# genomewalker/metadamage

Measured on AMD Instinct MI355X. Metric: TaxID damage fits/sec, higher is better.
Workload: dtype f64

## Files before the change

metadamage_amd/csrc/mdfit.hip:

```cpp
#include <hip/hip_runtime.h>

#include <algorithm>
#include <cmath>
#include <cstdint>
#include <cstdlib>
#include <cstdio>
#include <cstring>
#include <mutex>

#include "../../include/mdfit.h"
#include "mdfit_hpdi.h"
#include "mdfit_host.h"
#include "mdfit_laplace.h"
#include "mdfit_mappsis.h"
#include "mdfit_model.h"
#include "mdfit_primitive.h"
#include "mdfit_special.h"

#ifdef MDFIT_DEV_HPTIME
__device__ unsigned long long* g_dev_hpt = nullptr;
#define MDFIT_DEV_T(idx) \
  do {                     \
    if (g_dev_hpt != nullptr) g_dev_hpt[(idx)] = __builtin_amdgcn_s_memrealtime(); \
  } while (0)
#endif

namespace mdfit {

constexpr int kAll = 0, kFR = 1;

__device__ __forceinline__ double* diag(double* out, int64_t taxon, int sub) {
  return out + taxon * MDFIT_NOUT + MDFIT_F_DIAG + MDFIT_DIAG_STRIDE * sub;
}

__device__ __forceinline__ double sel4(const double v[4], int j) {
  return j == 0 ? v[0] : (j == 1 ? v[1] : (j == 2 ? v[2] : v[3]));
}

#ifdef MDFIT_STAMP
__device__ unsigned long long* g_stamp = nullptr;
__device__ __forceinline__ unsigned long long stamp() {
  __builtin_amdgcn_sched_barrier(0);
  unsigned long long t = __builtin_amdgcn_s_memtime();
  __builtin_amdgcn_sched_barrier(0);
  return t;
}
#endif

constexpr int kWsReady = 8, kWsClaim = 9, kWsStarted = 10, kWsBad = 11;
constexpr int kWsEarlyClaimed = 12;
constexpr int kWsDefRes = 32, kWsDefDone = 33, kWsDefClaim = 34, kWsEarlyQuit = 35;
constexpr unsigned kDefClosed = 0x40000000u;
constexpr int kReadyStride = 6;
static_assert(kReadyStride == MDFIT_NSUBFIT, "K0 zeroes the ready list with one thread per (taxon, sub-fit)");
__device__ __forceinline__ void ready_put(uint64_t* f, double v) {
  __hip_atomic_store(f, ~(uint64_t)__double_as_longlong(isnan(v) ? NAN : v), __ATOMIC_RELAXED,
                     __HIP_MEMORY_SCOPE_AGENT);
}
__device__ __forceinline__ uint64_t ready_get(const uint64_t* f) {
  return __hip_atomic_load(f, __ATOMIC_RELAXED, __HIP_MEMORY_SCOPE_AGENT);
}
constexpr int kHpdiCtr = 16;

__device__ __forceinline__ int kpos(int i) { return i < kNHalf ? i : i - kNHalf; }

__global__ __launch_bounds__(256) void init_kernel(const uint32_t* __restrict__ gy,
                                                   const uint32_t* __restrict__ gN, int64_t T,
                                                   double* __restrict__ out, int* __restrict__ ws) {
  const int64_t i = (int64_t)blockIdx.x * blockDim.x + threadIdx.x;
  if (i < 64) ws[i] = 0;
  if (i < MDFIT_NSUBFIT * T) reinterpret_cast<double*>(reinterpret_cast<char*>(ws) + 256)[i] = 0.0;
  if (i >= MDFIT_NSUBFIT * T) return;
  const int64_t taxon = i / MDFIT_NSUBFIT;
  const int sub = (int)(i % MDFIT_NSUBFIT);
  const bool pmd = sub == 0 || sub == 2 || sub == 3;
  const int lo = (sub == 3 || sub == 5) ? kNHalf : 0;
  const int hi = sub < 2 ? kNPos : lo + kNHalf;
  double s[8] = {0, 0, 0, 0, 0, 0, 0, 0};
  for (int c = lo; c < hi; ++c) {
    const double y = (double)gy[taxon * kLD + c], N = (double)gN[taxon * kLD + c];
    const int k = kpos(c);
    s[0] += y;
    s[1] += N;
    if (k == 0) { s[2] += y; s[3] += N; }
    if (k == 1) { s[4] += y; s[5] += N; }
    if (k >= 9) { s[6] += y; s[7] += N; }
  }
  double u0[4];
  u0[3] = flog(100.0);
  if (!pmd) {
    u0[0] = logit(clampd((s[0] + 0.5) / (s[1] + 1.0), 1e-4, 0.9));
    u0[1] = u0[2] = 0.0;
  } else {
    const double c0 = clampd((s[6] + 0.5) / (s[7] + 1.0), 1e-4, 0.3);
    const double r1 = (s[2] + 0.5) / (s[3] + 1.0);
    const double r2 = (s[4] + 0.5) / (s[5] + 1.0);
    const double A0 = clampd(r1 - c0, 1e-3, 0.9 * (1.0 - c0));
    double q0 = 1.0 / 3.0;
    if (r1 - c0 > 1e-3) q0 = clampd(1.0 - (r2 - c0) / (r1 - c0), 0.05, 0.95);
    u0[0] = logit(q0);
    u0[1] = logit(A0);
    u0[2] = c0;
  }
  double* dg = diag(out, taxon, sub);
#pragma unroll
  for (int j = 0; j < 4; ++j) dg[j] = u0[j];
}

#ifndef MDFIT_FIT_WAVES_PER_EU
#define MDFIT_FIT_WAVES_PER_EU 2
#endif


constexpr int kIdle = 0, kAllFit = 1, kPairFit = 2, kNextPair = 3;
constexpr int kPrioEvals = 15;

constexpr unsigned kEscIndef = 1u, kEscProbe = 2u, kEscNc = 4u, kEscExhOk = 8u, kEscN = 16u, kEscCount = 0x70u,
                   kEscRescued = 0x100u, kEscRelax = 0x200u, kEscPolish = 0x400u, kEscPolishProbe = 0x800u,
                   kEscGrad = 0x1000u, kEscGradProbe = 0x2000u, kEscGradN = 0x4000u, kEscGradCount = 0x3C000u;


struct HpdiIO {
  const uint32_t* gN;
// ... 38 lines not shown
  __shared__ int s_b[2];
  bool wide = false;
  hpdi::WideRec rec;
  if (valid) {
    double lo = NAN, hi = NAN;
    if (!skip) wide = !hpdi::prep_position(N, a, b, lo, hi, rec);
    if (!wide) hpdi_write<kFit>(io, item, N, lo, hi);
  }
  bool near = false;
  if (wide) {
    const double tau = sqrt(rec.sd * rec.sd + (rec.mu - rec.m) * (rec.mu - rec.m));
    near = rec.m < 1.5 * tau || rec.N - rec.m < 1.5 * tau;
  }
  const int w = (int)threadIdx.x / kWave, ln = (int)threadIdx.x % kWave;
  const unsigned long long mf = __ballot(wide && near), mb = __ballot(wide && !near);
  if (ln == 0) {
    s_n[0][w] = __popcll(mf);
    s_n[1][w] = __popcll(mb);
  }
  __syncthreads();
  if (threadIdx.x == 0) {
    int tf = 0, tb = 0;
#pragma unroll
    for (int k = 0; k < kW; ++k) {
      tf += s_n[0][k];
      tb += s_n[1][k];
    }
    s_b[0] = tf ? atomicAdd(ctr, tf) : 0;
    s_b[1] = tb ? atomicAdd(ctr + 2, tb) : 0;
  }
  __syncthreads();
  if (wide) {
    int bf = s_b[0], bb = s_b[1];
    for (int k = 0; k < w; ++k) {
      bf += s_n[0][k];
      bb += s_n[1][k];
    }
    rec.item = item;
    const unsigned long long below = (1ull << ln) - 1ull;
    const int64_t slot = near ? (int64_t)(bf + __popcll(mf & below)) : n_items - 1 - (bb + __popcll(mb & below));
    recs[slot] = rec;
  }
}

__device__ __forceinline__ double tree8(const double* x) {
  return ((x[0] + x[1]) + (x[2] + x[3])) + ((x[4] + x[5]) + (x[6] + x[7]));
}
__device__ __forceinline__ double tree16(const double* x) { return tree8(x) + tree8(x + 8); }

template <int PPL>
__global__ __launch_bounds__(kWave) __attribute__((amdgpu_waves_per_eu(MDFIT_FIT_WAVES_PER_EU)))
void fit_kernel(const uint32_t* __restrict__ gy, const uint32_t* __restrict__ gN, int64_t T,
                int max_iter, double tol, double* __restrict__ out, int* __restrict__ ws,
                double* __restrict__ ready, int base_prio) {
  static_assert(PPL == 1 || PPL == 2, "points per lane");
  constexpr int kSlot = PPL == 1 ? 32 : 16;
  constexpr int kHalf = kSlot / 2;
  const int lane = threadIdx.x;
  const int r = lane & (kSlot - 1);
  const int h = r / kHalf;
  const int jh = r & (kHalf - 1);
  const int leader = lane & ~(kSlot - 1);
  const unsigned long long slot_mask = (kSlot == 32 ? 0xFFFFFFFFull : 0xFFFFull) << leader;
  const int qi = blockIdx.x % kQueues;
  const int64_t tl = T * qi / kQueues, nq = T * (qi + 1) / kQueues - tl;

  PointData pa, pb;
  int vA_all, vA_pair, vB_all = 0, vB_pair = 0;
  int kA_all, kA_pair, kB_all = 0, kB_pair = 0, colA_all;
  if (PPL == 1) {
    const int i = r & 15;
    vA_all = vA_pair = i < kNHalf;
    kA_all = kA_pair = vA_all ? i : 0;
    colA_all = vA_all ? h * kNHalf + i : 0;
  } else {
    vA_all = vB_all = r < kNHalf;
    kA_all = kB_all = vA_all ? r : 0;
    colA_all = vA_all ? r : 0;
    kA_pair = 2 * jh;
    kB_pair = 2 * jh + 1;
    vA_pair = true;
    vB_pair = kB_pair < kNHalf;
    kB_pair = vB_pair ? kB_pair : 0;
  }
  const int srcA = leader + (PPL == 2 ? kA_pair : 0);
  const int srcB = leader + (PPL == 2 ? (vB_pair ? kB_pair : 0) : 0);
  pa.y = pa.N = pb.y = pb.N = 0.0;
  pa.valid = vA_all;
  pa.k = kA_all;
  pb.valid = vB_all;
  pb.k = kB_all;
  pa.pmd = pb.pmd = true;

  __shared__ __attribute__((aligned(16))) double sAcc[kNAcc][kWave + 2];
  __shared__ __attribute__((aligned(16))) double sSum[2][kWave];
  if (blockIdx.x == 0 && lane == 0)
    __hip_atomic_store(ws + kWsStarted, 1, __ATOMIC_RELAXED, __HIP_MEMORY_SCOPE_AGENT);
  int mode = kIdle;
  int drained = 0, allok = 0;
  int64_t taxon = 0;
  int sub = 0;
  int running = 0;
  double u[4] = {0, 0, 0, 0}, ut[4] = {0, 0, 0, 0}, d[4] = {0, 0, 0, 0};
  double curF = INFINITY, curMag = 0.0, curPg = 0.0, t = 1.0;
  double curG3 = 0.0, curGd = 0.0;
  unsigned esc = 0u;
  int evals = 0, status = MDFIT_MAXITER;
  int first = 1;
#ifdef MDFIT_STAMP
  unsigned long long st_eval = 0, st_red = 0, st_logic = 0, st_fetch = 0, st_trips = 0;
  unsigned long long st_claim1 = 0, st_claim2 = 0;
  const unsigned long long k0 = stamp();
#endif

  while (true) {
#ifdef MDFIT_STAMP
    const unsigned long long f0 = stamp();
#endif
    bool starting = false;
    const bool need1 = mode == kIdle && !drained;
#ifdef MDFIT_STAMP
    const unsigned long long a0 = stamp();
#endif
    if (__any(need1)) {
      const unsigned long long m = __ballot(need1 && r == 0);
      int base = 0;
      if (lane == 0) base = atomicAdd(ws + qi, __popcll(m));
      base = __shfl(base, 0);
      if (need1) {
        const int64_t task = (int64_t)base + __popcll(m & ((1ull << leader) - 1ull));
        if (task >= 2 * nq) {
          drained = true;
        } else {
          sub = task < nq ? 0 : 1;
          taxon = tl + task - (sub ? nq : 0);
          mode = kAllFit;
          starting = true;
          pa.pmd = pb.pmd = sub == 0;
          pa.valid = vA_all;
          pa.k = kA_all;
          pa.y = pa.valid ? (double)gy[taxon * kLD + colA_all] : 0.0;
          pa.N = pa.valid ? (double)gN[taxon * kLD + colA_all] : 0.0;
          if (PPL == 2) {
            pb.valid = vB_all;
            pb.k = kB_all;
            pb.y = pb.valid ? (double)gy[taxon * kLD + kNHalf + colA_all] : 0.0;
            pb.N = pb.valid ? (double)gN[taxon * kLD + kNHalf + colA_all] : 0.0;
          }
          const double* dg = diag(out, taxon, sub);
#pragma unroll
          for (int j = 0; j < 4; ++j) u[j] = dg[j];
        }
      }
    }
#ifdef MDFIT_STAMP
    const unsigned long long a1 = stamp();
#ifndef MDFIT_STAMP2
    st_claim1 += a1 - a0;
#endif
#endif
    const bool next = mode == kNextPair;
    if (__any(next)) {
      if (PPL == 2) {
        const double ya = __shfl(pa.y, srcA), Na = __shfl(pa.N, srcA);
        const double yb = __shfl(pb.y, srcA), Nb = __shfl(pb.N, srcA);
        const double ya2 = __shfl(pa.y, srcB), Na2 = __shfl(pa.N, srcB);
        const double yb2 = __shfl(pb.y, srcB), Nb2 = __shfl(pb.N, srcB);
        if (next) {
          pa.valid = vA_pair;
          pa.k = kA_pair;
          pa.y = h ? yb : ya;
          pa.N = h ? Nb : Na;
          pb.valid = vB_pair;
          pb.k = kB_pair;
          pb.y = vB_pair ? (h ? yb2 : ya2) : 0.0;
          pb.N = vB_pair ? (h ? Nb2 : Na2) : 0.0;
        }
      }
      if (next) {
        sub = (pa.pmd ? 2 : 4) + h;
        mode = kPairFit;
        starting = true;
        if (!allok) {
          const double* dg = diag(out, taxon, sub);
#pragma unroll
          for (int j = 0; j < 4; ++j) u[j] = dg[j];
        }
      }
    }
#if defined(MDFIT_STAMP) && !defined(MDFIT_STAMP2)
    st_claim2 += stamp() - a1;
#endif
    if (starting) {
#pragma unroll
      for (int j = 0; j < 4; ++j) ut[j] = u[j];
      curF = INFINITY;
      curMag = curPg = 0.0;
      esc = 0u;
      t = 1.0;
      evals = 0;
      status = MDFIT_MAXITER;
      first = true;
      running = true;
    }
    if (!__any(mode != kIdle || !drained)) break;
#ifdef MDFIT_STAMP
    const unsigned long long e0 = stamp();
#endif
    if (!__any(running)) continue;

    const bool whole = mode == kAllFit;
    const Theta th = make_theta<kHalf>(pa.pmd, ut);
    double acc[kNAcc];
#pragma unroll
    for (int j = 0; j < kNAcc; ++j) acc[j] = 0.0;
    const int accf = (esc & kEscPolish) != 0u;
    const bool null_wave = !__any(running && pa.pmd != 0);
    const bool whole_wave = !__any(running && !whole);
    if (PPL == 1) {
      point_accum<true>(pa, th, acc, accf, null_wave, whole_wave);
    } else {
      const bool src15 = whole || h == 1;
      auto pad3 = [&](const LG3& v) -> LG3 { return src15 ? rowb3<15>(v) : rowb3<7>(v); };
      const PointArgs gb = point_args(pb, th);
      const LG3 t3b = lg3<true>(pb.N + th.phi);
      const LG3 t6 = pad3(t3b);
      const LG3 tb1 = lg3<true>(pb.y + gb.a);
      const LG3 tb2 = lg3<true>(pb.N - pb.y + gb.b);
      LG3 tb4, tb5;
      if (null_wave) {
        tb4 = pad3(tb1);
        tb5 = pad3(tb2);
      } else {
        tb4 = lg3<true>(gb.a);
        tb5 = lg3<true>(gb.b);
      }
      double accb[kNAcc];
#pragma unroll
      for (int j = 0; j < kNAcc; ++j) accb[j] = 0.0;
      point_finish(pb, th, gb, tb1, tb2, t3b, tb4, tb5, t6, accb, accf);
      const PointArgs ga = point_args(pa, th);
      const LG3 ta3 = lg3<true>(pa.N + th.phi);
      const LG3 ta1 = lg3<true>(pa.y + ga.a);
      const LG3 ta2 = lg3<true>(pa.N - pa.y + ga.b);
      LG3 ta4 = tb4, ta5 = tb5;
      if (!null_wave && !whole_wave) {
        ta4 = lg3<true>(ga.a);
        ta5 = lg3<true>(ga.b);
      }
      point_finish(pa, th, ga, ta1, ta2, ta3, ta4, ta5, t6, acc, accf);
#pragma unroll
      for (int j = 0; j < kNAcc; ++j) acc[j] = opaque(acc[j]) + opaque(accb[j]);
    }
#ifdef MDFIT_STAMP
    const unsigned long long e1 = stamp();
#endif
#pragma unroll
    for (int j = 0; j < kNAcc; ++j) sAcc[j][lane] = acc[j];
    __syncthreads();
    if (PPL == 1) {
      const double* a = &sAcc[jh][leader + 16 * h];
      const double* b = &sAcc[jh][leader + 16 * (1 - h)];
      double x[16];
#pragma unroll
      for (int k = 0; k < 16; ++k) {
        const double ak = a[k], bk = b[k];
        x[k] = whole ? ak + bk : ak;
      }
      sSum[0][lane] = tree16(x);
      __syncthreads();
      const double* src = &sSum[0][leader + 16 * h];
#pragma unroll
      for (int j = 0; j < kNAcc; ++j) acc[j] = src[j];
// ... 165 lines not shown
                                                     : (i == 6 ? (double)status : ((esc & kEscPolish) ? 1.0 : 0.0))));
          diag(out, taxon, sub)[i] = v;
        }
        allok = status == MDFIT_OK;
        running = false;
      }
    }
    if (__any(running && evals >= 2 * kPrioEvals)) __builtin_amdgcn_s_setprio(3);
    else if (__any(running && evals >= kPrioEvals)) __builtin_amdgcn_s_setprio(2);
    else if (base_prio) __builtin_amdgcn_s_setprio(1);
    else __builtin_amdgcn_s_setprio(0);
    const unsigned long long busy = __ballot(running);
    if ((busy & slot_mask) == 0ull) {
      if (mode == kAllFit) {
        if (sub == 0) {
          auto sig = [](double v) {
            const double e = exp(-fabs(v));
            const double rr = rcp(1.0 + e);
            return v >= 0.0 ? rr : e * rr;
          };
          const bool badA = vA_all && pa.y > pa.N;
          const bool badB = PPL == 2 && vB_all && pb.y > pb.N;
          const bool bad = (__ballot(badA || badB) & slot_mask) != 0ull;
          if (r == 0) {
#ifdef MDFIT_DEV_HPTIME
            MDFIT_DEV_T(taxon);
#endif
            const int idx = atomicAdd(ws + kWsReady, 1);
            uint64_t* e = reinterpret_cast<uint64_t*>(ready + (int64_t)idx * kReadyStride);
            ready_put(e + 0, bad ? NAN : sig(u[0]));
            ready_put(e + 1, bad ? NAN : sig(u[1]));
            ready_put(e + 2, bad ? NAN : u[2]);
            ready_put(e + 3, bad ? NAN : exp(u[3]) + 2.0);
            __hip_atomic_store(e + 4, ~(uint64_t)taxon, __ATOMIC_RELAXED, __HIP_MEMORY_SCOPE_AGENT);
          }
        }
        mode = kNextPair;
      } else if (mode == kPairFit) {
#ifdef MDFIT_DEV_HPTIME
        if (r == 0) MDFIT_DEV_T(T + taxon);
#endif
        mode = kIdle;
      }
    }
#ifdef MDFIT_STAMP
    const unsigned long long l1 = stamp();
    st_fetch += e0 - f0;
    st_eval += e1 - e0;
    st_red += e2 - e1;
    st_logic += l1 - e2;
    st_trips += 1;
#endif
  }
#ifdef MDFIT_STAMP
  if (lane == 0 && g_stamp != nullptr) {
    unsigned long long* rr = g_stamp + (int64_t)blockIdx.x * 8;
    rr[0] = st_eval;
    rr[1] = st_red;
    rr[2] = st_logic;
    rr[3] = st_fetch;
    rr[4] = st_trips;
    rr[5] = stamp() - k0;
    rr[6] = st_claim1;
    rr[7] = st_claim2;
  }
#endif
}


__device__ __forceinline__ double predict_median(double A, double q, double c, int k, double N) {
  if (N == 0.0) return NAN;
  return fmin(fma(A, powk(1.0 - q, k), c), 1.0);
}

template <int G>
__device__ __forceinline__ double nsigma_group(bool valid, double lP, double lN, double n) {
  const double v = valid ? 1.0 : 0.0;
  const double dd0 = v * ((-2.0 * lP) - (-2.0 * lN));
  const double md = gsum<G>(dd0) / n;
  const double wP = gsum<G>(v * (-2.0 * lP));
  const double wN = gsum<G>(v * (-2.0 * lN));
  const double dd = v * (dd0 - md);
  const double var = gsum<G>(dd * dd) / n;
  return (wN - wP) / sqrt(n * var);
}

__device__ __forceinline__ Theta sel(bool c, const Theta& a, const Theta& b) {
  Theta r;
  r.q = c ? a.q : b.q;
  r.omq = c ? a.omq : b.omq;
  r.iomq = c ? a.iomq : b.iomq;
  r.A = c ? a.A : b.A;
  r.JA = c ? a.JA : b.JA;
  r.c = c ? a.c : b.c;
  r.iomc = c ? a.iomc : b.iomc;
  r.delta = c ? a.delta : b.delta;
  r.phi = c ? a.phi : b.phi;
  r.lprior = c ? a.lprior : b.lprior;
  return r;
}

__device__ __forceinline__ double read_lane(double v, int l) {
  return __hiloint2double(__builtin_amdgcn_readlane(__double2hiint(v), l),
                          __builtin_amdgcn_readlane(__double2loint(v), l));
}
__device__ __forceinline__ Theta read_theta(const Theta& t, int l) {
// ... 512 lines not shown
    }
  }
}

__global__ __launch_bounds__(kWave) void objective_kernel(
    const int32_t* __restrict__ model, const int32_t* __restrict__ subset,
    const uint32_t* __restrict__ gy, const uint32_t* __restrict__ gN, const double* __restrict__ gu,
    int64_t n, double* __restrict__ F, double* __restrict__ g, double* __restrict__ H,
    double* __restrict__ ell_out) {
  const int64_t i = blockIdx.x;
  if (i >= n) return;
  if (threadIdx.x < kNPos) ell_out[i * kNPos + threadIdx.x] = 0.0;
  __syncthreads();
  double u[4];
#pragma unroll
  for (int j = 0; j < 4; ++j) u[j] = gu[i * 4 + j];
  const bool pmd = model[i] == 0;
  if (subset[i] == 0) objective_group<kAll>(gy, gN, i, pmd, false, u, F, g, H, ell_out);
  else objective_group<kFR>(gy, gN, i, pmd, subset[i] == 2, u, F, g, H, ell_out);
}

}

namespace mdfit::host {
thread_local char g_err[512] = "";

int set_err(int code, const char* msg) {
  std::snprintf(g_err, sizeof(g_err), "%s", msg);
  return code;
}

int check_launch(const char* what) {
  hipError_t e = hipGetLastError();
  if (e != hipSuccess) {
    std::snprintf(g_err, sizeof(g_err), "%s: %s", what, hipGetErrorString(e));
    return (int)e;
  }
  g_err[0] = '\0';
  return 0;
}
}

namespace {
using mdfit::host::check_launch;
using mdfit::host::fit_grid;
using mdfit::host::g_err;
using mdfit::host::set_err;

constexpr int kProfMax = 256;
constexpr int64_t kPpl2MinTaxa = 13000;
constexpr int64_t kStreamMaxTaxa = 60000;
constexpr int64_t kDeferCap = 131072;
int64_t defer_cap(int64_t n_taxa) { return std::min<int64_t>(n_taxa * mdfit::kNPos, kDeferCap); }
struct ProfState {
  bool on = false;
  bool fit_only = false;
  int n = 0;
  hipEvent_t ev[kProfMax][4];
  bool made = false;
};
ProfState g_prof;

void prof_record(int slot, hipStream_t s) {
  if (g_prof.fit_only && (slot == 0 || slot == 3)) return;
  if (g_prof.on && g_prof.n < kProfMax) (void)hipEventRecord(g_prof.ev[g_prof.n][slot], s);
}
}

namespace {
int env_int(const char* name, int dflt) {
  const char* e = std::getenv(name);
  return e ? std::atoi(e) : dflt;
}

double* ready_buf(void* ws) { return reinterpret_cast<double*>(static_cast<char*>(ws) + 256); }
mdfit::hpdi::WideRec* hpdi_recs(void* ws) {
  return reinterpret_cast<mdfit::hpdi::WideRec*>(static_cast<char*>(ws) + 256);
}
mdfit::hpdi::WideRec* hpdi_recs_after_ready(void* ws, int64_t n_taxa) {
  return reinterpret_cast<mdfit::hpdi::WideRec*>(static_cast<char*>(ws) + 256 +
                                                 n_taxa * mdfit::kReadyStride * (int64_t)sizeof(double));
}

struct Fork {
  hipStream_t s[2] = {nullptr, nullptr};
  hipEvent_t fork[2] = {nullptr, nullptr}, join[2] = {nullptr, nullptr};
  bool ok = false;
  std::mutex mu;
};
Fork* side_fork() {
  constexpr int kMaxDev = 64;
  static Fork f[kMaxDev];
  static std::mutex make_mu;
  int dev = 0;
  if (hipGetDevice(&dev) != hipSuccess || dev < 0 || dev >= kMaxDev) return nullptr;
  Fork& x = f[dev];
  std::lock_guard<std::mutex> g(make_mu);
  if (!x.ok) {
    bool ok = true;
    for (int k = 0; k < 2 && ok; ++k)
      ok = (x.s[k] != nullptr || hipStreamCreateWithFlags(&x.s[k], hipStreamNonBlocking) == hipSuccess) &&
           (x.fork[k] != nullptr || hipEventCreateWithFlags(&x.fork[k], hipEventDisableTiming) == hipSuccess) &&
           (x.join[k] != nullptr || hipEventCreateWithFlags(&x.join[k], hipEventDisableTiming) == hipSuccess);
    if (!ok) return nullptr;
    x.ok = true;
  }
// ... 50 lines not shown
#endif

int mdfit_profile_enable(int on) {
  if (on && !g_prof.made) {
    for (int i = 0; i < kProfMax; ++i)
      for (int j = 0; j < 4; ++j)
        if (hipEventCreate(&g_prof.ev[i][j]) != hipSuccess) return set_err(MDFIT_E_HIP, "hipEventCreate");
    g_prof.made = true;
  }
  g_prof.on = on != 0;
  g_prof.fit_only = on == 2;
  g_prof.n = 0;
  return 0;
}

int mdfit_profile_read(double* call_ms, double* fit_ms, int32_t* n_calls) {
  if (!call_ms || !fit_ms || !n_calls) return set_err(MDFIT_E_ARG, "null argument");
  double a = 0.0, b = 0.0;
  for (int i = 0; i < g_prof.n; ++i) {
    float x = 0.f, y = 0.f;
    if (hipEventSynchronize(g_prof.ev[i][2]) != hipSuccess ||
        (!g_prof.fit_only && (hipEventSynchronize(g_prof.ev[i][3]) != hipSuccess ||
                              hipEventElapsedTime(&x, g_prof.ev[i][0], g_prof.ev[i][3]) != hipSuccess)) ||
        hipEventElapsedTime(&y, g_prof.ev[i][1], g_prof.ev[i][2]) != hipSuccess)
      return set_err(MDFIT_E_HIP, "hipEventElapsedTime");
    a += x;
    b += y;
  }
  *call_ms = g_prof.fit_only ? -1.0 : a;
  *fit_ms = b;
  *n_calls = g_prof.n;
  g_prof.n = 0;
  return 0;
}

void mdfit_default_opts(mdfit_opts* o) {
  if (!o) return;
  std::memset(o, 0, sizeof(*o));
  o->mode = MDFIT_MODE_MAP;
  o->max_iter = 200;
  o->tol_step = 1e-9;
  o->seed = 0;
  o->num_warmup = 500;
  o->num_samples = 1000;
  o->index_base = 0;
}

int64_t mdfit_workspace_bytes(int64_t n_taxa, const mdfit_opts* opts) {
  if (n_taxa < 0) return 0;
  mdfit_opts o;
  mdfit_default_opts(&o);
  if (opts) o = *opts;
  if (o.mode == MDFIT_MODE_NUTS) return mdfit::nuts::workspace_bytes(n_taxa, o.num_samples);
  return 256 + n_taxa * mdfit::kReadyStride * (int64_t)sizeof(double) +
         (n_taxa >= kStreamMaxTaxa ? n_taxa * mdfit::kNPos * (int64_t)sizeof(mdfit::hpdi::WideRec) : 0) +
         defer_cap(n_taxa) * (int64_t)sizeof(int);
}

int mdfit_fit_batch(const uint32_t* y, const uint32_t* N, const uint32_t* mm, int64_t n_taxa,
                    const mdfit_opts* opts, double* out, float* pred, int32_t* status,
                    void* workspace, void* hip_stream) {
  if (n_taxa < 0) return set_err(MDFIT_E_ARG, "n_taxa < 0");
  if (n_taxa == 0) return 0;
  if (!y || !N || !out || !status) return set_err(MDFIT_E_ARG, "null required pointer");
  if (!workspace) return set_err(MDFIT_E_ARG, "workspace (mdfit_workspace_bytes() bytes) required");
  mdfit_opts o;
  mdfit_default_opts(&o);
  if (opts) o = *opts;
  if (o.mode != MDFIT_MODE_MAP && o.mode != MDFIT_MODE_NUTS) return set_err(MDFIT_E_ARG, "unsupported mode");
  if (o.max_iter < 1) return set_err(MDFIT_E_ARG, "max_iter < 1");
  if (n_taxa > ((int64_t)1 << 25)) return set_err(MDFIT_E_ARG, "n_taxa exceeds 2^25 per call");
  hipStream_t s = (hipStream_t)hip_stream;
  int* ws = (int*)workspace;
  prof_record(0, s);
  if (o.mode == MDFIT_MODE_NUTS) {
    if (hipMemsetAsync(ws, 0, 256, s) != hipSuccess) return check_launch("hipMemsetAsync(workspace)");
    if (int rc = mdfit::nuts::fit_batch(y, N, mm, n_taxa, o, out, pred, status, workspace, s)) return rc;
    prof_record(3, s);
    if (g_prof.on && g_prof.n < kProfMax) ++g_prof.n;
    return 0;
  }
  const int64_t n_init = MDFIT_NSUBFIT * n_taxa;
  mdfit::host::debug_poison(s);
  hipLaunchKernelGGL(mdfit::init_kernel, dim3((unsigned)((n_init + 255) / 256)), dim3(256), 0, s, y, N,
                     n_taxa, out, ws);
  if (int rc = check_launch("init_kernel")) return rc;
  int ppl = n_taxa >= kPpl2MinTaxa ? 2 : 1;
  if (const char* e = std::getenv("MDFIT_FIT_PPL")) ppl = std::atoi(e) == 2 ? 2 : 1;
  const int per = pred != nullptr ? mdfit::kNPos : 1;
  const int64_t n_items = n_taxa * per;
  double* ready = ready_buf(workspace);
  Fork* fk = side_fork();
  std::unique_lock<std::mutex> fork_lock;
  if (fk != nullptr) fork_lock = std::unique_lock<std::mutex>(fk->mu);
  bool stream = n_taxa < kStreamMaxTaxa;
  if (const char* e = std::getenv("MDFIT_HPDI_STREAM")) stream = stream || std::atoi(e) != 0;
  const int early_per_cu =
      (fk != nullptr && stream) ? env_int("MDFIT_STREAM_WAVES_PER_CU", MDFIT_STREAM_WAVES_PER_CU) : 0;
  int* defer = reinterpret_cast<int*>(static_cast<char*>(workspace) + mdfit_workspace_bytes(n_taxa, &o) -
                                      defer_cap(n_taxa) * (int64_t)sizeof(int));
  const uint32_t defer_ticks = (uint32_t)std::max(0, env_int("MDFIT_STREAM_DEFER_US", 1000)) * 100u;
  ForkScope fork_hp(early_per_cu > 0 ? fk : nullptr, s, 0);
  if (early_per_cu > 0) {
    const int64_t g = std::min<int64_t>(fit_grid(mdfit::hpdi_stream_kernel<true>, n_items, mdfit::kWave, early_per_cu),
                                        kDeferCap / mdfit::kWave);
    hipLaunchKernelGGL(mdfit::hpdi_stream_kernel<true>, dim3((unsigned)g), dim3(mdfit::kWave), 0, fork_hp.side(), N,
                       n_taxa, per, out, pred, ws, (const double*)ready, defer, defer_ticks);
    if (int rc = check_launch("hpdi_stream_kernel")) return rc;
  }
  prof_record(1, s);
  {
    const int fit_prio = env_int("MDFIT_FIT_BASE_PRIO", 1) != 0 ? 1 : 0;
    int occ = 8;
    const int cap_env = env_int("MDFIT_FIT_WAVES_PER_CU", 0);
    if (ppl == 2) {
      if (hipOccupancyMaxActiveBlocksPerMultiprocessor(&occ, mdfit::fit_kernel<2>, mdfit::kWave, 0) != hipSuccess) occ = 8;
      const int cap = cap_env > 0 ? cap_env : std::max(1, occ - early_per_cu);
      const int64_t g = fit_grid(mdfit::fit_kernel<2>, 2 * n_taxa, 4, cap);
      hipLaunchKernelGGL(mdfit::fit_kernel<2>, dim3((unsigned)g), dim3(mdfit::kWave), 0, s, y, N, n_taxa,
                         o.max_iter, o.tol_step, out, ws, ready, fit_prio);
    } else {
      if (hipOccupancyMaxActiveBlocksPerMultiprocessor(&occ, mdfit::fit_kernel<1>, mdfit::kWave, 0) != hipSuccess) occ = 8;
      const int cap = cap_env > 0 ? cap_env : std::max(1, occ - early_per_cu);
      const int64_t g = fit_grid(mdfit::fit_kernel<1>, 2 * n_taxa, 2, cap);
      hipLaunchKernelGGL(mdfit::fit_kernel<1>, dim3((unsigned)g), dim3(mdfit::kWave), 0, s, y, N, n_taxa,
                         o.max_iter, o.tol_step, out, ws, ready, fit_prio);
    }
  }
  if (int rc = check_launch("fit_kernel")) return rc;
  prof_record(2, s);
  ForkScope fork_as(fk, s, 1);
  const bool asm_main = stream;
  const hipStream_t s_asm = asm_main ? s : fork_as.side();
  const hipStream_t s_hp = asm_main ? fork_as.side() : s;
  mdfit::host::debug_poison(s_asm);
  hipLaunchKernelGGL(mdfit::assemble_kernel, dim3((unsigned)n_taxa), dim3(mdfit::kWave), 0, s_asm, y, N,
                     mm, n_taxa, out, pred, status);
  if (int rc = check_launch("assemble_kernel")) return rc;
  if (stream) {
    const int64_t g = fit_grid(mdfit::hpdi_stream_kernel<false>, n_items, mdfit::kWave,
                               env_int("MDFIT_HPDI_WAVES_PER_CU", 0));
    mdfit::host::debug_poison(s_hp);
    hipLaunchKernelGGL(mdfit::hpdi_stream_kernel<false>, dim3((unsigned)g), dim3(mdfit::kWave), 0, s_hp, N, n_taxa, per,
                       out, pred, ws, (const double*)ready, defer, defer_ticks);
    if (int rc = check_launch("hpdi_stream_kernel")) return rc;
  } else {
    mdfit::HpdiIO io{};
    io.gN = N;
    io.ready = ready;
    io.out = out;
    io.pred = pred;
    io.per = per;
    if (int rc = launch_hpdi<true>(io, n_items, ws + mdfit::kHpdiCtr, hpdi_recs_after_ready(workspace, n_taxa), s))
      return rc;
  }
  if (int rc = fork_as.join()) return rc;
  if (int rc = fork_hp.join()) return rc;
  prof_record(3, s);
  if (g_prof.on && g_prof.n < kProfMax) ++g_prof.n;
  return 0;
}

int mdfit_noise(const uint32_t* y, const uint32_t* N, const uint32_t* mm, int64_t n_taxa, double* out,
                void* hip_stream) {
  if (n_taxa < 0 || (n_taxa > 0 && (!y || !N || !mm || !out))) return set_err(MDFIT_E_ARG, "bad arguments");
  if (n_taxa == 0) return 0;
  hipLaunchKernelGGL(mdfit::noise_kernel, dim3((unsigned)n_taxa), dim3(mdfit::kWave), 0, (hipStream_t)hip_stream, y,
                     N, mm, n_taxa, out);
  return check_launch("noise_kernel");
}

int mdfit_betabinom_logpmf(const double* y, const double* N, const double* alpha,
                           const double* beta, int64_t n, double* out, double* grad,
                           void* hip_stream) {
  if (n < 0 || (n > 0 && (!y || !N || !alpha || !beta || !out)))
    return set_err(MDFIT_E_ARG, "bad arguments");
  if (n == 0) return 0;
  const unsigned blocks = (unsigned)((n + 255) / 256);
  hipLaunchKernelGGL(mdfit::betabinom_kernel, dim3(blocks), dim3(256), 0,
// ... 216 lines not shown
```

metadamage_amd/csrc/mdfit_model.h:

```cpp
#pragma once

#include <hip/hip_runtime.h>

#include <type_traits>

#include "../../include/mdfit.h"
#include "mdfit_special.h"

namespace mdfit {

constexpr int kNPos = MDFIT_NPOS;
constexpr int kNHalf = MDFIT_NHALF;
constexpr int kLD = MDFIT_LD;
constexpr int kNMM = MDFIT_NMM;

constexpr double kULo[4] = {-25.0, -25.0, 0.0, -25.0};
constexpr double kUHi[4] = {25.0, 25.0, 0.999, 20.0};
constexpr double kEpsAct = 1e-8;
constexpr double kNoiseF = 1.4e-14;
constexpr double kPgTol = 1e-6;
constexpr double kQuadK = 10.0;

template <int Ctrl>
__device__ __forceinline__ double dpp(double v) {
  const int lo = __builtin_amdgcn_mov_dpp(__double2loint(v), Ctrl, 0xF, 0xF, false);
  const int hi = __builtin_amdgcn_mov_dpp(__double2hiint(v), Ctrl, 0xF, 0xF, false);
  return __hiloint2double(hi, lo);
}

template <int G>
__device__ __forceinline__ double gsum(double v) {
  static_assert(G == 2 || G == 4 || G == 8 || G == 16 || G == 32 || G == 64, "group size");
  asm volatile("" : "+v"(v));
  if (G >= 2) v += dpp<0xB1>(v);
  if (G >= 4) v += dpp<0x4E>(v);
  if (G >= 8) v += dpp<0x141>(v);
  if (G >= 16) v += dpp<0x140>(v);
  if (G >= 32) v += __shfl_xor(v, 16, 64);
  if (G >= 64) v += __shfl_xor(v, 32, 64);
  return v;
}

__device__ __forceinline__ double opaque(double v) {
  asm volatile("" : "+v"(v));
  return v;
}

__device__ __forceinline__ double clampd(double x, double lo, double hi) {
  return fmin(fmax(x, lo), hi);
}
__device__ __forceinline__ double logit(double p) { return flog(p) - flog1p(-p); }

__device__ __forceinline__ void logit_parts(double u, double& p, double& omp, double& lp,
                                            double& l1mp) {
  const double e = exp(-fabs(u));
  const double r = rcp(1.0 + e);
  const double sp = flog1p(e);
  const bool pos = u >= 0.0;
  p = pos ? r : e * r;
  omp = pos ? e * r : r;
  lp = pos ? -sp : u - sp;
  l1mp = pos ? -(u + sp) : -sp;
}

__device__ __forceinline__ double xrow(double v) {
  const unsigned lo = (unsigned)__double2loint(v), hi = (unsigned)__double2hiint(v);
  const auto rl = __builtin_amdgcn_permlane16_swap(lo, lo, false, false);
  const auto rh = __builtin_amdgcn_permlane16_swap(hi, hi, false, false);
  const bool odd = (threadIdx.x & 16) != 0;
  return __hiloint2double((int)(odd ? rh[0] : rh[1]), (int)(odd ? rl[0] : rl[1]));
}

template <int N>
__device__ __forceinline__ double rowb(double v) {
  return dpp<0x150 + N>(v);
}

struct Theta {
  double q, omq, iomq;
  double A, JA;
  double c, iomc;
  double delta, phi;
  double lprior;
};

template <int W = 16>
__device__ __forceinline__ Theta make_theta(bool pmd, const double u[4]) {
  static_assert(W == 16 || W == 8, "row width");
  const int i = (int)(threadIdx.x & (W - 1));
  const bool hi8 = W == 8 && (threadIdx.x & 8);
  const double v = i == 0 ? u[0] : u[1];
  const double e = exp(i < 2 ? -fabs(v) : u[3]);
  const double sp = flog1p(i < 2 ? e : -u[2]);
  const double rr = rcp(1.0 + e);
  const bool pos = v >= 0.0;
  const double p = pos ? rr : e * rr, omp = pos ? e * rr : rr;
  const double lpp = (pos ? -sp : v - sp) + 2.0 * (pos ? -(v + sp) : -sp);
  auto bc = [=](double x, auto n) {
    constexpr int N = decltype(n)::value;
    if constexpr (W == 16) return rowb<N>(x);
    else return hi8 ? rowb<8 + N>(x) : rowb<N>(x);
  };
  using I0 = std::integral_constant<int, 0>;
  using I1 = std::integral_constant<int, 1>;
  using I2 = std::integral_constant<int, 2>;
  Theta th;
  th.q = bc(p, I0{});
  th.omq = bc(omp, I0{});
  const double lpq = bc(lpp, I0{});
  const double A = bc(p, I1{}), omA = bc(omp, I1{}), lpA = bc(lpp, I1{});
  th.delta = bc(e, I2{});
  const double l1mc = bc(sp, I2{});
  th.iomq = rcp(th.omq);
  th.phi = th.delta + 2.0;
  th.lprior = lpq - th.delta / 1000.0;
  if (pmd) {
    th.A = A;
    th.JA = A * omA;
    th.c = u[2];
    th.iomc = rcp(1.0 - th.c);
    th.lprior += lpA + 8.0 * l1mc;
  } else {
    th.A = th.JA = th.c = 0.0;
// ... 71 lines not shown
  const double lFF = fma(D * D, Qa, fma(omD * omD, Qb, S1));
  if (pd.valid) {
    const double lDDq = lDD * Dq, lDDA = lDD * DA;
    acc[0] += ell;
    acc[1] += mag;
    acc[2] = fma(lD, Dq, acc[2]);
    acc[3] = fma(lD, DA, acc[3]);
    acc[4] = fma(lD, Dc, acc[4]);
    acc[5] += lF;
    acc[6] = fma(lDDq, Dq, fma(lD, Dqq, acc[6]));
    acc[7] = fma(lDDq, DA, fma(lD, DqA, acc[7]));
    acc[8] = fma(lDDq, Dc, acc[8]);
    acc[9] = fma(lDF, Dq, acc[9]);
    acc[10] = fma(lDDA, DA, acc[10]);
    acc[11] = fma(lDDA, Dc, acc[11]);
    acc[12] = fma(lDF, DA, acc[12]);
    acc[13] = fma(lDD * Dc, Dc, acc[13]);
    acc[14] = fma(lDF, Dc, acc[14]);
    acc[15] += lFF;
  }
  return ell;
}

template <int N>
__device__ __forceinline__ LG3 rowb3(const LG3& t) {
  return {rowb<N>(t.l), rowb<N>(t.p), rowb<N>(t.q)};
}

template <bool kRowPhi = false>
__device__ __forceinline__ double point_accum(const PointData& pd, const Theta& th, double acc[kNAcc],
                                              int accf = 0, bool null_row = false, bool whole_pair = false) {
  const PointArgs pa = point_args(pd, th);
  const LG3 t3 = lg3<true>(pd.N + th.phi);
  const LG3 t6 = kRowPhi ? rowb3<15>(t3) : lg3<true>(th.phi);
  const LG3 t1 = lg3<true>(pd.y + pa.a);
  const LG3 t2 = lg3<true>(pd.N - pd.y + pa.b);
  LG3 t4, t5;
  if (kRowPhi && null_row) {
    t4 = rowb3<15>(t1);
    t5 = rowb3<15>(t2);
  } else if (kRowPhi && whole_pair) {
    const bool odd = (threadIdx.x & 16) != 0;
    const LG3 mine = lg3<true>(odd ? pa.b : pa.a);
    const LG3 other = {xrow(mine.l), xrow(mine.p), xrow(mine.q)};
    t4 = odd ? other : mine;
    t5 = odd ? mine : other;
  } else {
    t4 = lg3<true>(pa.a);
    t5 = lg3<true>(pa.b);
  }
  return point_finish(pd, th, pa, t1, t2, t3, t4, t5, t6, acc, accf);
}

__device__ __forceinline__ double point_ell(double y, double N, double D, double phi) {
  return bb_logpmf(y, N, D, phi);
}

struct Eval {
  double F, mag;
  double g[4];
  double H[10];
};

__device__ __forceinline__ int hidx(int j, int m) {
  return j == 0 ? m : (j == 1 ? 3 + m : (j == 2 ? 5 + m : 9));
}

__device__ __forceinline__ void finish_eval(bool pmd, const Theta& th, const double s[kNAcc],
                                            Eval& e) {
#pragma clang fp contract(off)
  const double q = th.q, A = th.A, c = th.c, delta = th.delta;
  const double J[4] = {q * th.omq, th.JA, 1.0, delta};
  const double J2[4] = {J[0] * fma(-2.0, q, 1.0), th.JA * fma(-2.0, A, 1.0), 0.0, delta};
  const double gp[4] = {fma(-3.0, q, 1.0), pmd ? fma(-3.0, A, 1.0) : 0.0, pmd ? -8.0 * th.iomc : 0.0,
                        0.0 - delta / 1000.0};
  const double hp[4] = {-3.0 * J[0], pmd ? -3.0 * th.JA : 0.0,
                        pmd ? -8.0 * th.iomc * th.iomc : 0.0, 0.0 - delta / 1000.0};
  const bool infeasible = pmd && (A + c >= 1.0);
  e.F = infeasible ? INFINITY : -(s[0] + th.lprior);
  e.mag = s[1];
#pragma unroll
  for (int j = 0; j < 4; ++j) {
    const bool fixed = !pmd && (j == 1 || j == 2);
    e.g[j] = fixed ? 0.0 : -(j == 2 ? fma(-8.0, th.iomc, s[2 + j]) : fma(J[j], s[2 + j], gp[j]));
  }
#pragma unroll
  for (int j = 0; j < 4; ++j) {
#pragma unroll
    for (int m = j; m < 4; ++m) {
      const int k = hidx(j, m);
      double h = J[j] * s[6 + k] * J[m];
      if (j == m) {
        const double dg = fma(J2[j], s[2 + j], hp[j]);
        h = j == 2 ? s[6 + k] + dg : fma(J[j] * s[6 + k], J[m], dg);
      }
      const bool fixed = !pmd && (j == 1 || j == 2 || m == 1 || m == 2);
      e.H[k] = fixed ? 0.0 : -h;
    }
  }
}

__device__ __forceinline__ double maxabs4(const double v[4]) {
  return fmax(fmax(fabs(v[0]), fabs(v[1])), fmax(fabs(v[2]), fabs(v[3])));
}

__device__ __forceinline__ double pgnorm(const double u[4], const double g[4]) {
// ... 279 lines not shown
```

metadamage_amd/engine.py:

```python

from __future__ import annotations

import ctypes
import os
from dataclasses import dataclass

import numpy as np

from . import _lib


def _torch():
    import torch

    if not torch.cuda.is_available():
        raise _lib.MdfitError("no HIP device available: the mdfit engine runs on MI355X only")
    return torch


def _stream_handle(torch, stream=None) -> ctypes.c_void_p:
    s = stream if stream is not None else torch.cuda.current_stream()
    return ctypes.c_void_p(s.cuda_stream)


@dataclass
class FitBatch:

    out: "object"
    pred: "object"
    status: "object"
    workspace: "object" = None
    lap: "object" = None
    diag: "object" = None
    summ: "object" = None
    loo: "object" = None
    psis: "object" = None


def to_device_counts(y, N, mm=None, device="cuda"):
    torch = _torch()
    y = np.ascontiguousarray(y, dtype=np.uint32)
    N = np.ascontiguousarray(N, dtype=np.uint32)
    if y.ndim != 2 or y.shape[1] != _lib.LD or N.shape != y.shape:
        raise ValueError(f"y, N must be uint32[T][{_lib.LD}], got {y.shape} / {N.shape}")
    ty = torch.from_numpy(y.view(np.int32)).to(device)
    tN = torch.from_numpy(N.view(np.int32)).to(device)
    tm = None
    if mm is not None:
        mm = np.ascontiguousarray(mm, dtype=np.uint32)
        if mm.shape != (y.shape[0], _lib.NPOS, _lib.NMM):
            raise ValueError(f"mm must be uint32[T][30][12], got {mm.shape}")
        tm = torch.from_numpy(mm.view(np.int32)).to(device)
    return ty, tN, tm


def alloc_outputs(n_taxa: int, device="cuda", with_pred: bool = True, opts: _lib.MdfitOpts | None = None) -> FitBatch:
    torch = _torch()
    out = torch.empty((n_taxa, _lib.NOUT), dtype=torch.float64, device=device)
    pred = (
        torch.empty((n_taxa, _lib.NPRED, _lib.NPOS), dtype=torch.float32, device=device)
        if with_pred
        else None
    )
    status = torch.empty((n_taxa,), dtype=torch.int32, device=device)
    return FitBatch(out, pred, status, alloc_workspace(n_taxa, device, opts))


def workspace_bytes(n_taxa: int, opts: _lib.MdfitOpts | None = None) -> int:
    lib = _lib.load()
    return int(lib.mdfit_workspace_bytes(int(n_taxa), ctypes.byref(opts) if opts is not None else None))


def alloc_workspace(n_taxa: int, device="cuda", opts: _lib.MdfitOpts | None = None):
    torch = _torch()
    return torch.empty((workspace_bytes(n_taxa, opts),), dtype=torch.uint8, device=device)


def samples_view(res: FitBatch, n_taxa: int, opts: _lib.MdfitOpts):
    torch = _torch()
    S = int(opts.num_samples)
    n = n_taxa * 6 * S * 4
    return res.workspace[_lib.SAMPLES_OFFSET:_lib.SAMPLES_OFFSET + 8 * n].view(torch.float64).view(n_taxa, 6, S, 4)


def fit_batch_device(ty, tN, tm=None, opts: _lib.MdfitOpts | None = None, res: FitBatch | None = None,
                     stream=None) -> FitBatch:
    torch = _torch()
    lib = _lib.load()
    T = int(ty.shape[0])
    for name, t in (("y", ty), ("N", tN)):
        if not (t.is_cuda and t.is_contiguous() and t.dtype == torch.int32 and tuple(t.shape) == (T, _lib.LD)):
            raise ValueError(f"{name} must be a contiguous cuda int32/uint32 view of shape [T, {_lib.LD}]")
    if tm is not None and not (tm.is_cuda and tm.is_contiguous() and tm.numel() == T * _lib.NPOS * _lib.NMM):
        raise ValueError("mm must be a contiguous cuda tensor of T*30*12 uint32")
    if res is None:
        res = alloc_outputs(T, device=ty.device, opts=opts)
    o = opts if opts is not None else _lib.default_opts()
    if res.workspace is None or res.workspace.numel() < workspace_bytes(T, o):
        res.workspace = alloc_workspace(T, ty.device, o)
    _lib.check(
        lib.mdfit_fit_batch(
            ctypes.c_void_p(ty.data_ptr()),
            ctypes.c_void_p(tN.data_ptr()),
            ctypes.c_void_p(tm.data_ptr()) if tm is not None else None,
            T,
            ctypes.byref(o),
            ctypes.c_void_p(res.out.data_ptr()),
            ctypes.c_void_p(res.pred.data_ptr()) if res.pred is not None else None,
            ctypes.c_void_p(res.status.data_ptr()),
            ctypes.c_void_p(res.workspace.data_ptr()),
            _stream_handle(torch, stream),
        )
    )
    return res


def map_laplace_device(ty, tN, res: FitBatch, lap=None, gh=None, stream=None, u=None):
    torch = _torch()
    lib = _lib.load()
    T = int(ty.shape[0])
    if lap is None:
        lap = torch.empty((T, 3, _lib.NLAPLACE), dtype=torch.float64, device=ty.device)
    for name, t, n in (("lap", lap, T * 3 * _lib.NLAPLACE), ("gh", gh, T * 3 * 20), ("u", u, T * 3 * 4)):
        if t is not None and not (t.is_cuda and t.is_contiguous() and t.dtype == torch.float64 and t.numel() == n):
            raise ValueError(f"{name} must be a contiguous cuda float64 tensor of {n} elements")
    if not (res.out.is_contiguous() and res.status.is_contiguous() and int(res.out.shape[0]) == T):
        raise ValueError("res must hold the contiguous records of these T taxa")
    args = [ctypes.c_void_p(ty.data_ptr()), ctypes.c_void_p(tN.data_ptr()), ctypes.c_void_p(res.out.data_ptr()),
# ... 742 lines not shown
```

Before: 9.934 million.

## Use idle wave half as helper for solo fits and park new claims

In the PPL=1 fit kernel, when only one 32-lane half of a wave is still running a fit, the idle half now mirrors the active half's data via permlane32 swaps. It computes half of the lgamma evaluations so the active half does fewer per iteration. It also parks new task claims in a half whose partner half has been running long (evals >= threshold), so long fits can be helped instead of being restarted alongside new ones. This adds cross-lane swaps, extra selects, register pressure and a global atomic stats counter in the workspace, and parking may reduce throughput by idling lanes.

After: 9.963 million, median of 4. No clear change (+0.3%).

```diff
diff --git a/metadamage_amd/csrc/mdfit.hip b/metadamage_amd/csrc/mdfit.hip
--- a/metadamage_amd/csrc/mdfit.hip
+++ b/metadamage_amd/csrc/mdfit.hip
@@ -66,9 +66,11 @@
 
 __global__ __launch_bounds__(256) void init_kernel(const uint32_t* __restrict__ gy,
                                                    const uint32_t* __restrict__ gN, int64_t T,
-                                                   double* __restrict__ out, int* __restrict__ ws) {
+                                                   double* __restrict__ out, int* __restrict__ ws,
+                                                   unsigned long long* __restrict__ solo_stats) {
   const int64_t i = (int64_t)blockIdx.x * blockDim.x + threadIdx.x;
   if (i < 64) ws[i] = 0;
+  if (i == 0) *solo_stats = 0ull;
   if (i < MDFIT_NSUBFIT * T) reinterpret_cast<double*>(reinterpret_cast<char*>(ws) + 256)[i] = 0.0;
   if (i >= MDFIT_NSUBFIT * T) return;
   const int64_t taxon = i / MDFIT_NSUBFIT;
@@ -213,7 +215,8 @@
 __global__ __launch_bounds__(kWave) __attribute__((amdgpu_waves_per_eu(MDFIT_FIT_WAVES_PER_EU)))
 void fit_kernel(const uint32_t* __restrict__ gy, const uint32_t* __restrict__ gN, int64_t T,
                 int max_iter, double tol, double* __restrict__ out, int* __restrict__ ws,
-                double* __restrict__ ready, int base_prio) {
+                double* __restrict__ ready, int base_prio, int park,
+                unsigned long long* __restrict__ solo_stats) {
   static_assert(PPL == 1 || PPL == 2, "points per lane");
   constexpr int kSlot = PPL == 1 ? 32 : 16;
   constexpr int kHalf = kSlot / 2;
@@ -268,6 +271,12 @@
   unsigned esc = 0u;
   int evals = 0, status = MDFIT_MAXITER;
   int first = 1;
+  auto vreg = [](int v) {
+    asm volatile("" : "+v"(v));
+    return v;
+  };
+  int n_solo = 0, n_parked = 0;
+  const int park_evals = park < 0 ? -park : park;
 #ifdef MDFIT_STAMP
   unsigned long long st_eval = 0, st_red = 0, st_logic = 0, st_fetch = 0, st_trips = 0;
   unsigned long long st_claim1 = 0, st_claim2 = 0;
@@ -279,7 +288,13 @@
     const unsigned long long f0 = stamp();
 #endif
     bool starting = false;
-    const bool need1 = mode == kIdle && !drained;
+    bool need1 = mode == kIdle && !drained;
+    if (PPL == 1 && park_evals > 0 && __any(need1)) {
+      const unsigned long long lm = __ballot(running && evals >= park_evals);
+      const bool parked = need1 && (lm & ~slot_mask) != 0ull;
+      n_parked = vreg(n_parked + (parked ? 1 : 0));
+      need1 = need1 && !parked;
+    }
 #ifdef MDFIT_STAMP
     const unsigned long long a0 = stamp();
 #endif
@@ -371,6 +386,23 @@
     if (!__any(running)) continue;
 
     const bool whole = mode == kAllFit;
+    const unsigned long long run_m = __ballot(running);
+    const bool solo = PPL == 1 && park > 0 && ((run_m & 0xFFFFFFFFull) != 0ull) != ((run_m >> 32) != 0ull);
+    const int helper = vreg(solo && (run_m & slot_mask) == 0ull ? 1 : 0);
+    if (PPL == 1 && solo) {
+      const double xy = xhalf(pa.y), xN = xhalf(pa.N);
+      const int xp = xhalf(pa.pmd);
+      pa.y = helper ? xy : pa.y;
+      pa.N = helper ? xN : pa.N;
+      pa.pmd = helper ? xp : pa.pmd;
+      pa.valid = helper ? 0 : pa.valid;
+#pragma unroll
+      for (int j = 0; j < 4; ++j) {
+        const double x = xhalf(ut[j]);
+        ut[j] = helper ? x : ut[j];
+      }
+      n_solo = vreg(n_solo + 1);
+    }
     const Theta th = make_theta<kHalf>(pa.pmd, ut);
     double acc[kNAcc];
 #pragma unroll
@@ -379,7 +411,7 @@
     const bool null_wave = !__any(running && pa.pmd != 0);
     const bool whole_wave = !__any(running && !whole);
     if (PPL == 1) {
-      point_accum<true>(pa, th, acc, accf, null_wave, whole_wave);
+      point_accum_wide(pa, th, acc, accf, solo, helper, null_wave, whole_wave);
     } else {
       const bool src15 = whole || h == 1;
       auto pad3 = [&](const LG3& v) -> LG3 { return src15 ? rowb3<15>(v) : rowb3<7>(v); };
@@ -651,6 +683,11 @@
     st_trips += 1;
 #endif
   }
+  if (PPL == 1) {
+    const int np = n_parked + xhalf(n_parked);
+    if (lane == 0 && (n_solo | np) != 0)
+      atomicAdd(solo_stats, ((unsigned long long)(unsigned)np << 32) | (unsigned)n_solo);
+  }
 #ifdef MDFIT_STAMP
   if (lane == 0 && g_stamp != nullptr) {
     unsigned long long* rr = g_stamp + (int64_t)blockIdx.x * 8;
@@ -1269,6 +1306,15 @@
 constexpr int64_t kStreamMaxTaxa = 60000;
 constexpr int64_t kDeferCap = 131072;
 int64_t defer_cap(int64_t n_taxa) { return std::min<int64_t>(n_taxa * mdfit::kNPos, kDeferCap); }
+int64_t map_core_bytes(int64_t n_taxa) {
+  return 256 + n_taxa * mdfit::kReadyStride * (int64_t)sizeof(double) +
+         (n_taxa >= kStreamMaxTaxa ? n_taxa * mdfit::kNPos * (int64_t)sizeof(mdfit::hpdi::WideRec) : 0) +
+         defer_cap(n_taxa) * (int64_t)sizeof(int);
+}
+int64_t solo_stats_offset(int64_t n_taxa) { return (map_core_bytes(n_taxa) + 127) / 128 * 128; }
+#ifndef MDFIT_FIT_PARK_EVALS
+#define MDFIT_FIT_PARK_EVALS 20
+#endif
 struct ProfState {
   bool on = false;
   bool fit_only = false;
@@ -1425,9 +1471,7 @@
   mdfit_default_opts(&o);
   if (opts) o = *opts;
   if (o.mode == MDFIT_MODE_NUTS) return mdfit::nuts::workspace_bytes(n_taxa, o.num_samples);
-  return 256 + n_taxa * mdfit::kReadyStride * (int64_t)sizeof(double) +
-         (n_taxa >= kStreamMaxTaxa ? n_taxa * mdfit::kNPos * (int64_t)sizeof(mdfit::hpdi::WideRec) : 0) +
-         defer_cap(n_taxa) * (int64_t)sizeof(int);
+  return solo_stats_offset(n_taxa) + 128;
 }
 
 int mdfit_fit_batch(const uint32_t* y, const uint32_t* N, const uint32_t* mm, int64_t n_taxa,
@@ -1454,9 +1498,11 @@
     return 0;
   }
   const int64_t n_init = MDFIT_NSUBFIT * n_taxa;
+  unsigned long long* solo_stats =
+      reinterpret_cast<unsigned long long*>(static_cast<char*>(workspace) + solo_stats_offset(n_taxa));
   mdfit::host::debug_poison(s);
   hipLaunchKernelGGL(mdfit::init_kernel, dim3((unsigned)((n_init + 255) / 256)), dim3(256), 0, s, y, N,
-                     n_taxa, out, ws);
+                     n_taxa, out, ws, solo_stats);
   if (int rc = check_launch("init_kernel")) return rc;
   int ppl = n_taxa >= kPpl2MinTaxa ? 2 : 1;
   if (const char* e = std::getenv("MDFIT_FIT_PPL")) ppl = std::atoi(e) == 2 ? 2 : 1;
@@ -1470,7 +1516,7 @@
   if (const char* e = std::getenv("MDFIT_HPDI_STREAM")) stream = stream || std::atoi(e) != 0;
   const int early_per_cu =
       (fk != nullptr && stream) ? env_int("MDFIT_STREAM_WAVES_PER_CU", MDFIT_STREAM_WAVES_PER_CU) : 0;
-  int* defer = reinterpret_cast<int*>(static_cast<char*>(workspace) + mdfit_workspace_bytes(n_taxa, &o) -
+  int* defer = reinterpret_cast<int*>(static_cast<char*>(workspace) + map_core_bytes(n_taxa) -
                                       defer_cap(n_taxa) * (int64_t)sizeof(int));
   const uint32_t defer_ticks = (uint32_t)std::max(0, env_int("MDFIT_STREAM_DEFER_US", 1000)) * 100u;
   ForkScope fork_hp(early_per_cu > 0 ? fk : nullptr, s, 0);
@@ -1486,18 +1532,20 @@
     const int fit_prio = env_int("MDFIT_FIT_BASE_PRIO", 1) != 0 ? 1 : 0;
     int occ = 8;
     const int cap_env = env_int("MDFIT_FIT_WAVES_PER_CU", 0);
+    const int park_evals = ppl == 1 ? std::max(0, env_int("MDFIT_FIT_PARK_EVALS", MDFIT_FIT_PARK_EVALS)) : 0;
+    const int park = env_int("MDFIT_FIT_WIDE", 1) != 0 ? park_evals : -park_evals;
     if (ppl == 2) {
       if (hipOccupancyMaxActiveBlocksPerMultiprocessor(&occ, mdfit::fit_kernel<2>, mdfit::kWave, 0) != hipSuccess) occ = 8;
       const int cap = cap_env > 0 ? cap_env : std::max(1, occ - early_per_cu);
       const int64_t g = fit_grid(mdfit::fit_kernel<2>, 2 * n_taxa, 4, cap);
       hipLaunchKernelGGL(mdfit::fit_kernel<2>, dim3((unsigned)g), dim3(mdfit::kWave), 0, s, y, N, n_taxa,
-                         o.max_iter, o.tol_step, out, ws, ready, fit_prio);
+                         o.max_iter, o.tol_step, out, ws, ready, fit_prio, park, solo_stats);
     } else {
       if (hipOccupancyMaxActiveBlocksPerMultiprocessor(&occ, mdfit::fit_kernel<1>, mdfit::kWave, 0) != hipSuccess) occ = 8;
       const int cap = cap_env > 0 ? cap_env : std::max(1, occ - early_per_cu);
       const int64_t g = fit_grid(mdfit::fit_kernel<1>, 2 * n_taxa, 2, cap);
       hipLaunchKernelGGL(mdfit::fit_kernel<1>, dim3((unsigned)g), dim3(mdfit::kWave), 0, s, y, N, n_taxa,
-                         o.max_iter, o.tol_step, out, ws, ready, fit_prio);
+                         o.max_iter, o.tol_step, out, ws, ready, fit_prio, park, solo_stats);
     }
   }
   if (int rc = check_launch("fit_kernel")) return rc;
diff --git a/metadamage_amd/csrc/mdfit_model.h b/metadamage_amd/csrc/mdfit_model.h
--- a/metadamage_amd/csrc/mdfit_model.h
+++ b/metadamage_amd/csrc/mdfit_model.h
@@ -69,6 +69,18 @@
   const auto rh = __builtin_amdgcn_permlane16_swap(hi, hi, false, false);
   const bool odd = (threadIdx.x & 16) != 0;
   return __hiloint2double((int)(odd ? rh[0] : rh[1]), (int)(odd ? rl[0] : rl[1]));
+}
+
+__device__ __forceinline__ double xhalf(double v) {
+  const unsigned lo = (unsigned)__double2loint(v), hi = (unsigned)__double2hiint(v);
+  const auto rl = __builtin_amdgcn_permlane32_swap(lo, lo, false, false);
+  const auto rh = __builtin_amdgcn_permlane32_swap(hi, hi, false, false);
+  const bool up = (threadIdx.x & 32) != 0;
+  return __hiloint2double((int)(up ? rh[0] : rh[1]), (int)(up ? rl[0] : rl[1]));
+}
+__device__ __forceinline__ int xhalf(int v) {
+  const auto r = __builtin_amdgcn_permlane32_swap((unsigned)v, (unsigned)v, false, false);
+  return (int)((threadIdx.x & 32) != 0 ? r[0] : r[1]);
 }
 
 template <int N>
@@ -246,6 +258,45 @@
   return point_finish(pd, th, pa, t1, t2, t3, t4, t5, t6, acc, accf);
 }
 
+__device__ __forceinline__ double point_accum_wide(const PointData& pd, const Theta& th, double acc[kNAcc], int accf,
+                                                   bool solo, bool helper, bool null_row, bool whole_pair) {
+#pragma clang fp contract(off)
+  const PointArgs pa = point_args(pd, th);
+  const bool odd = (threadIdx.x & 16) != 0;
+  const double xb = pd.N - pd.y + pa.b;
+  const double xab = (whole_pair && !odd) ? pa.a : pa.b;
+  double x1 = pd.N + th.phi, x2 = pd.y + pa.a;
+  if (solo) {
+    x1 = helper ? xb : x1;
+    x2 = helper ? xab : x2;
+  }
+  const LG3 t3 = lg3<true>(x1);
+  const LG3 t1 = lg3<true>(x2);
+  const LG3 t6 = rowb3<15>(t3);
+  LG3 t2, h2, t4, t5;
+  if (solo) {
+    t2 = {xhalf(t3.l), xhalf(t3.p), xhalf(t3.q)};
+    h2 = {xhalf(t1.l), xhalf(t1.p), xhalf(t1.q)};
+  } else {
+    t2 = lg3<true>(xb);
+  }
+  if (null_row) {
+    t4 = rowb3<15>(t1);
+    t5 = rowb3<15>(t2);
+  } else {
+    if (!solo) h2 = lg3<true>(xab);
+    if (whole_pair) {
+      const LG3 other = {xrow(h2.l), xrow(h2.p), xrow(h2.q)};
+      t4 = odd ? other : h2;
+      t5 = odd ? h2 : other;
+    } else {
+      t4 = lg3<true>(pa.a);
+      t5 = h2;
+    }
+  }
+  return point_finish(pd, th, pa, t1, t2, t3, t4, t5, t6, acc, accf);
+}
+
 __device__ __forceinline__ double point_ell(double y, double N, double D, double phi) {
   return bb_logpmf(y, N, D, phi);
 }
diff --git a/metadamage_amd/engine.py b/metadamage_amd/engine.py
--- a/metadamage_amd/engine.py
+++ b/metadamage_amd/engine.py
@@ -74,6 +74,13 @@
 def alloc_workspace(n_taxa: int, device="cuda", opts: _lib.MdfitOpts | None = None):
     torch = _torch()
     return torch.empty((workspace_bytes(n_taxa, opts),), dtype=torch.uint8, device=device)
+
+
+def fit_solo_counters(res: FitBatch, n_taxa: int) -> tuple[int, int]:
+    torch = _torch()
+    off = workspace_bytes(n_taxa) - 128
+    w = res.workspace[off:off + 8].view(torch.int32).cpu().numpy().view("uint32")
+    return int(w[0]), int(w[1])
 
 
 def samples_view(res: FitBatch, n_taxa: int, opts: _lib.MdfitOpts):
```
